# 0xPolygonZero/proof-protocol-decoder

Hardware: NVIDIA B200
Metric: mpt_nodes_keccak_hashed_per_sec (higher is better)
Workload: dtype u64

## Files before the change

proof_protocol_decoder_b200/csrc/gpu_dump.cu:

```cuda
#include "host_pipeline.h"

namespace ppd {

struct LitPool {
  std::vector<uint8_t> b;
  void u8(uint8_t v) { b.push_back(v); }
  void u32(uint32_t v) {
    uint8_t t[4];
    memcpy(t, &v, 4);
    b.insert(b.end(), t, t + 4);
  }
  void raw(const uint8_t* p, size_t n) {
    if (n) b.insert(b.end(), p, p + n);
  }
  void span(Span s) {
    u32(s.n);
    raw(s.p, s.n);
  }
  void u256(uint64_t v) {
    uint8_t be[32];
    memset(be, 0, 32);
    for (int i = 0; i < 8; i++) be[31 - i] = (uint8_t)(v >> (8 * i));
    raw(be, 32);
  }
// ... 88 lines not shown
      t += p.touched.size();
    }
  }
  memcpy(h + o_tb, touched_begin.data(), 4 * (n_ir + 1));
  memcpy(h + o_sa, seg_a.data(), 4 * n_seg);
  memcpy(h + o_sb, seg_b.data(), 4 * n_seg);
  memcpy(h + o_sg, seg_begin.data(), 4 * (n_ir + 1));
  L->d_plan.reserve(4 * o_end);
  uint32_t* d = L->d_plan.as<uint32_t>();
  CUDA_OK(cudaMemcpyAsync(d, h, 4 * o_base, cudaMemcpyHostToDevice, L->st));
  IrDumpPlanView P{};
  P.touched = d + o_touched, P.touched_begin = d + o_tb, P.seg_a = d + o_sa, P.seg_b = d + o_sb, P.seg_begin = d + o_sg;
  P.ir_base = reinterpret_cast<const uint64_t*>(d + o_base);
  P.seg_off = d + o_soff, P.ir_size = d + o_isz, P.ir_flag = d + o_ifl, P.ir_nuniq = d + o_inu;
  P.u_node = d + o_un, P.u_size = d + o_us, P.u_off = d + o_uo;
  pt.lap("  d:plan");
  launch_ir_size(L->last_view, P, n_ir, L->st);
  CUDA_OK(cudaGetLastError());
  CUDA_OK(cudaMemcpyAsync(h + o_soff, d + o_soff, 4 * (o_inu - o_soff), cudaMemcpyDeviceToHost, L->st));
  lane_sync(L);
  L->stats.h2d_bytes += 4.0 * o_base, L->stats.d2h_bytes += 4.0 * (o_inu - o_soff), L->stats.kernel_launches += 1;
  pt.lap("  d:size");
  const uint32_t *seg_off = h + o_soff, *ir_size = h + o_isz;
  uint32_t* ir_flag = h + o_ifl;
  std::vector<Out> host_parts(n_ir);
  Stamp st;
  uint64_t* ir_base = reinterpret_cast<uint64_t*>(h + o_base);
  uint64_t total = 8;
  for (uint32_t i = 0; i < n_ir; i++) {
    ir_base[i] = total;
// ... 91 lines not shown
```

proof_protocol_decoder_b200/csrc/gpu_txn.cu:

```cuda
#include "host_pipeline.h"
#include "txn_tables.h"

namespace ppd {

bool gpu_txn_enabled() {
#ifdef PPD_HOSTPROF
  return false;
#else
  return gpu_parse_enabled() && gpu_dump_enabled() && getenv("PPD_HOST_TXN") == nullptr;
#endif
}

struct LoopBatcher {
  static const int MAX_STREAMS = 16, BMAX = (int)LOOP_BATCH_MAX;
  struct Req {
    txn::LoopTask task;
    uint32_t n_txns = 0;
    cudaEvent_t ready = nullptr, start = nullptr, done = nullptr, done_blocking = nullptr;
    bool launched = false;
    uint32_t launches = 0;
    cudaError_t err = cudaSuccess;
  };
  struct LoopStream {
    cudaStream_t st = nullptr;
// ... 371 lines not shown
    P.ir_nuniq = cv.take<uint32_t>(n_ir + 1);
    d_big_off = cv.take<uint64_t>(n_ir + 1), d_big_cap = cv.take<uint32_t>(n_ir + 1);
    P.big_scratch = cv.take<uint32_t>(big_words + 16);
    P.u_node = cv.take<uint32_t>((size_t)n_touched + 16), P.u_size = cv.take<uint32_t>((size_t)n_touched + 16), P.u_off = cv.take<uint32_t>((size_t)n_touched + 16);
  };
  {
    Carve2 sz{nullptr};
    plan_layout(sz);
    L->d_plan.reserve(sz.off + 256);
    Carve2 cv{L->d_plan.as<uint8_t>()};
    plan_layout(cv);
  }
  P.ir_size = d_ir_size, P.ir_flag = d_ir_size + n_ir;
  P.touched = d_touched, P.touched_begin = d_touched_begin, P.seg_a = d_seg_a, P.seg_b = d_seg_b, P.seg_c = d_seg_c, P.seg_begin = d_seg_begin;
  P.seg_end = d_seg_end;
  P.big_off = d_big_off, P.big_cap = d_big_cap;
  P.flat = d_flat, P.lit = d_lit, P.ir_base = d_ir_base;
  auto up = [&](void* dst, const void* src, size_t bytes) {
    if (!bytes) return;
    lane_copy(L, dst, src, bytes);
    L->stats.h2d_bytes += (double)bytes;
  };
  up(d_txns, T.txns.data(), sizeof(txn::TxnDesc) * T.txns.size());
  up(d_seg_a, T.seg_a.data(), 4ull * n_seg), up(d_seg_b, T.seg_b.data(), 4ull * n_seg), up(d_seg_c, T.seg_c.data(), 4ull * n_seg);
  up(d_touched_begin, T.touched_begin.data(), 4ull * (n_ir + 1));
  if (!n_dummies) up(d_seg_begin, T.seg_begin.data(), 4ull * (n_ir + 1)), up(d_seg_end, T.seg_end.data(), 4ull * (n_ir + 1));
  up(d_lit, T.lit.data(), T.lit.size());
  up(d_big_off, big_off.data(), 8ull * n_ir), up(d_big_cap, big_cap.data(), 4ull * n_ir);
  up(v.key_pool + H.B.txn_key_base, T.txn_keys.data(), T.txn_keys.size());
  lane_copy_flush(L);
  CUDA_OK(cudaMemsetAsync(d_touched, 0xff, 4ull * n_touched, st));
// ... 242 lines not shown
```

proof_protocol_decoder_b200/csrc/ppd_dump.cu:

```cuda
#include <cstddef>
#include <cstdint>

#include "../../include/ppd_flat.h"
#include "arena.h"
#include "ppd_kernels.h"

namespace ppd {

namespace {

constexpr uint32_t HASH_ID_BASE = 0x80000000u;
constexpr uint32_t SET_CAP = 8192, MAX_UNIQ = 4096, NOT_FOUND = 0xffffffffu, UNSET = 0xffffffffu;
#ifndef PPD_DUMP_THREADS
#define PPD_DUMP_THREADS 1024
#endif
constexpr int DUMP_THREADS = PPD_DUMP_THREADS;

struct SharedSet {
  uint32_t key[SET_CAP];
  uint32_t slot[SET_CAP];
  uint32_t u_node[MAX_UNIQ], u_size[MAX_UNIQ], u_off[MAX_UNIQ];
  uint32_t u_par[MAX_UNIQ];
};
struct Set {
  uint32_t *key, *slot, *u_node, *u_size, *u_off, *u_par;
  uint32_t shift, mask, max_uniq;
  uint32_t n_uniq, n_done, flag;
};

__device__ __forceinline__ uint32_t hash_slot(const Set& s, uint32_t id) { return (id * 2654435761u) >> s.shift; }

__device__ __forceinline__ uint32_t set_find(const Set& s, uint32_t id) {
  uint32_t h = hash_slot(s, id);
  for (;;) {
    uint32_t k = s.key[h];
    if (k == id) return s.slot[h];
    if (k == NODE_EMPTY) return NOT_FOUND;
    h = (h + 1) & s.mask;
  }
}

__device__ void set_bind(Set& s, SharedSet& sm, const IrDumpPlanView& P, uint32_t ir, uint32_t tb) {
  if (threadIdx.x == 0) {
    const uint64_t big = P.big_off ? P.big_off[ir] : ~0ull;
    if (big == ~0ull) {
      s.key = sm.key, s.slot = sm.slot, s.u_node = sm.u_node, s.u_size = sm.u_size, s.u_off = sm.u_off, s.u_par = sm.u_par;
      s.mask = SET_CAP - 1, s.shift = 19, s.max_uniq = MAX_UNIQ;
    } else {
      const uint32_t cap = P.big_cap[ir];
      s.key = P.big_scratch + big, s.slot = s.key + cap, s.u_par = s.slot + cap;
      s.u_node = P.u_node + tb, s.u_size = P.u_size + tb, s.u_off = P.u_off + tb;
      s.mask = cap - 1, s.shift = 32 - (31 - __clz(cap)), s.max_uniq = cap / 2;
    }
  }
  __syncthreads();
}

__device__ __forceinline__ bool is_hash_id(uint32_t id) { return id >= HASH_ID_BASE && id != NODE_EMPTY; }
__device__ __forceinline__ uint32_t node_kind(const ArenaView& A, uint32_t id) { return A.nodes[id].w0 & 0xff; }

__device__ __forceinline__ uint32_t u256_sig(const uint8_t* be) {
  uint32_t i = 0;
  while (i < 32 && be[i] == 0) i++;
  return 32 - i;
}
__device__ __forceinline__ uint32_t u256_str_len(const uint8_t* be, uint32_t sig) { return sig == 0 ? 1u : (sig == 1 && be[31] < 0x80) ? 1u : 1u + sig; }
__device__ __forceinline__ uint32_t account_rlp_len(const AccountRec& r) {
  return 2 + u256_str_len(r.nonce, u256_sig(r.nonce)) + u256_str_len(r.balance, u256_sig(r.balance)) + 66;
}

__device__ __forceinline__ uint32_t child_size(const ArenaView& A, const Set& s, uint32_t c, uint32_t* flag) {
  if (c == NODE_EMPTY) return 1;
  if (is_hash_id(c)) return 33;
  uint32_t k = set_find(s, c);
  if (k != NOT_FOUND) return s.u_size[k];
  if (A.ref_len[c] != 32 && node_kind(A, c) != NK_ROOT) *flag = 1;
  return 33;
}

// ... 15 lines not shown
      for (uint32_t j = 0; j < k; j++) {
        uint32_t cs = child_size(A, s, A.child_pool[r.a0 + j], flag);
        if (cs == UNSET) return UNSET;
        total += cs;
      }
      return total;
    }
    default:
      *flag = 1;
      return 33;
  }
}

__device__ void build_set(Set& s, const uint32_t* ids, uint32_t n, const ArenaView& A, bool dedupe) {
  for (uint32_t i = threadIdx.x; i <= s.mask; i += blockDim.x) s.key[i] = NODE_EMPTY;
  if (threadIdx.x == 0) s.n_uniq = 0, s.n_done = 0, s.flag = 0;
  __syncthreads();
  for (uint32_t i = threadIdx.x; i < n; i += blockDim.x) {
    uint32_t id = ids[i];
    if (id == NODE_EMPTY || is_hash_id(id)) continue;
    if (dedupe && node_kind(A, id) == NK_ROOT) continue;
    uint32_t h = hash_slot(s, id);
    for (;;) {
      uint32_t prev = atomicCAS(&s.key[h], NODE_EMPTY, id);
      if (prev == NODE_EMPTY) {
        uint32_t k = dedupe ? atomicAdd(&s.n_uniq, 1u) : i;
        if (k < s.max_uniq) {
          s.slot[h] = k;
          s.u_node[k] = id;
        } else {
          s.flag = 1;
          s.slot[h] = 0;
        }
        break;
      }
      if (prev == id) break;
      h = (h + 1) & s.mask;
    }
  }
  __syncthreads();
}

}

__global__ void __launch_bounds__(DUMP_THREADS) ir_size_kernel(ArenaView A, IrDumpPlanView P) {
  extern __shared__ uint8_t smem_raw[];
  __shared__ Set s;
  const uint32_t ir = blockIdx.x;
  const uint32_t tb = P.touched_begin[ir], tn = P.touched_begin[ir + 1] - tb;
  set_bind(s, *reinterpret_cast<SharedSet*>(smem_raw), P, ir, tb);
  build_set(s, P.touched + tb, tn, A, true);
  const uint32_t nu = min(s.n_uniq, s.max_uniq);
  constexpr uint32_t PLACED = 0x80000000u, NO_KIDS = 0x40000000u;
  for (uint32_t k = threadIdx.x; k < nu; k += blockDim.x) s.u_par[k] = UNSET;
  __syncthreads();
  {
    uint32_t local_flag = 0;
    for (uint32_t k = threadIdx.x; k < nu; k += blockDim.x) {
      const NodeRec r = A.nodes[s.u_node[k]];
      const uint32_t kind = r.w0 & 0xff, nlen = (r.w0 >> 16) & 0xff;
      uint32_t fixed = 0, pend = 0;
      auto child = [&](uint32_t c) {
        if (c == NODE_EMPTY) return 1u;
        if (is_hash_id(c)) return 33u;
        const uint32_t kc = set_find(s, c);
        if (kc != NOT_FOUND) {
          if (atomicCAS(&s.u_par[kc], UNSET, k) != UNSET) local_flag = 1;
          pend++;
          return 0u;
        }
        if (A.ref_len[c] != 32 && node_kind(A, c) != NK_ROOT) local_flag = 1;
        return 33u;
      };
      switch (kind) {
        case NK_LEAF:
          fixed = 1 + 1 + nlen + 4 + r.a2;
          break;
        case NK_LEAF_ACCOUNT:
          fixed = 1 + 1 + nlen + 4 + account_rlp_len(A.accounts[r.a1]);
          break;
        case NK_EXT:
          fixed = 1 + 1 + nlen + child(r.a1);
          break;
        case NK_BRANCH: {
          const uint32_t mask = r.a1 & 0xffff, nk = __popc(mask);
          uint32_t cid[16];
#pragma unroll
          for (uint32_t j = 0; j < 16; j++) cid[j] = j < nk ? A.child_pool[r.a0 + j] : NODE_EMPTY;
          fixed = 1 + (16 - nk) + 4;
#pragma unroll
          for (uint32_t j = 0; j < 16; j++)
            if (j < nk) fixed += child(cid[j]);
          break;
        }
        default:
          local_flag = 1;
          fixed = 33;
      }
      s.u_size[k] = fixed;
      s.u_off[k] = pend ? pend : NO_KIDS;
    }
    if (local_flag) s.flag = 1;
  }
  __syncthreads();
  for (uint32_t k = threadIdx.x; k < nu; k += blockDim.x) {
    if (s.u_off[k] != NO_KIDS) continue;
    uint32_t cur = k;
    for (uint32_t guard = 0; guard < 128; guard++) {
      const uint32_t p = s.u_par[cur];
      if (p == UNSET) break;
      atomicAdd(&s.u_size[p], *reinterpret_cast<volatile uint32_t*>(&s.u_size[cur]));
      __threadfence_block();
      if (atomicSub(&s.u_off[p], 1u) != 1u) break;
      __threadfence_block();
      cur = p;
// ... 60 lines not shown
      if (q < se) {
        P.seg_off[q] = off;
        if (trie_slot != NOT_FOUND && atomicCAS(&s.u_off[trie_slot], UNSET, off) != UNSET) s.flag = 1;
      }
      __syncthreads();
      if (threadIdx.x == DUMP_THREADS - 1) scan_carry = off + sz;
      __syncthreads();
    }
    if (threadIdx.x == 0) {
      P.ir_size[ir] = scan_carry;
      s.n_done = 0;
    }
  }
  __syncthreads();
  if (!s.flag) {
    for (uint32_t k = threadIdx.x; k < nu; k += blockDim.x) {
      const NodeRec r = A.nodes[s.u_node[k]];
      const uint32_t kind = r.w0 & 0xff, nlen = (r.w0 >> 16) & 0xff;
      if (kind == NK_EXT) {
        const uint32_t c = is_hash_id(r.a1) ? NOT_FOUND : set_find(s, r.a1);
        if (c != NOT_FOUND) {
          if (s.u_off[c] != UNSET) s.flag = 1;
          s.u_off[c] = 2 + nlen;
        }
      } else if (kind == NK_BRANCH) {
        const uint32_t mask = r.a1 & 0xffff, nk = __popc(mask);
        uint32_t cid[16];
#pragma unroll
        for (uint32_t j = 0; j < 16; j++) cid[j] = j < nk ? A.child_pool[r.a0 + j] : NODE_EMPTY;
        uint32_t off = 1;
        for (uint32_t i = 0, j = 0; i < 16; i++) {
          if (!(mask & (1u << i))) {
            off += 1;
            continue;
          }
          uint32_t c_id = NODE_EMPTY;
#pragma unroll
          for (uint32_t z = 0; z < 16; z++)
            if (z == j) c_id = cid[z];
          j++;
          const uint32_t c = is_hash_id(c_id) ? NOT_FOUND : set_find(s, c_id);
          if (c != NOT_FOUND) {
            if (s.u_off[c] != UNSET) s.flag = 1;
            s.u_off[c] = off;
            off += s.u_size[c];
          } else {
            off += 33;
          }
        }
      }
    }
  }
  __syncthreads();
  for (int round = 0; round < 130; round++) {
    __syncthreads();
    if (s.flag || s.n_done >= nu) break;
    __syncthreads();
    uint32_t progressed = 0;
    for (uint32_t k = threadIdx.x; k < nu; k += blockDim.x) {
      if (*reinterpret_cast<volatile uint32_t*>(&s.u_size[k]) & PLACED) continue;
      const uint32_t p = s.u_par[k];
      uint32_t off = *reinterpret_cast<volatile uint32_t*>(&s.u_off[k]);
      if (p != UNSET) {
// ... 31 lines not shown
  const uint32_t w[8] = {x.x, x.y, x.z, x.w, y.x, y.y, y.z, y.w};
  uint32_t S[10];
  S[0] = (uint32_t)PPD_NODE_HASH | (w[0] << 8);
#pragma unroll
  for (int k = 1; k < 8; k++) S[k] = __funnelshift_r(w[k - 1], w[k], 24);
  S[8] = w[7] >> 24;
  S[9] = 0;
  const uint32_t head = (4u - (uint32_t)(reinterpret_cast<uintptr_t>(q) & 3u)) & 3u;
  for (uint32_t i = 0; i < head; i++) q[i] = (uint8_t)(S[0] >> (8 * i));
  uint32_t* qw = reinterpret_cast<uint32_t*>(q + head);
  const uint32_t sh = 8 * head, nwords = (33u - head) >> 2;
#pragma unroll
  for (int j = 0; j < 8; j++)
    if ((uint32_t)j < nwords) qw[j] = __funnelshift_r(S[j], S[j + 1], sh);
  const uint32_t done = head + 4 * nwords;
  for (uint32_t i = done; i < 33; i++) q[i] = (uint8_t)(S[i >> 2] >> (8 * (i & 3)));
  return q + 33;
}
__device__ __forceinline__ uint8_t* put_hash(uint8_t* q, const uint8_t* h32) {
  const uint4* src = reinterpret_cast<const uint4*>(h32);
  return put_hash_regs(q, __ldg(src), __ldg(src + 1));
}
__device__ __forceinline__ uint8_t* put_u32(uint8_t* q, uint32_t v) {
  q[0] = (uint8_t)v, q[1] = (uint8_t)(v >> 8), q[2] = (uint8_t)(v >> 16), q[3] = (uint8_t)(v >> 24);
  return q + 4;
}
__device__ __forceinline__ uint8_t* put_nibbles(uint8_t* q, const ArenaView& A, const NodeRec& r) {
  const uint32_t start = (r.w0 >> 8) & 0xff, n = (r.w0 >> 16) & 0xff;
  const uint8_t* key = A.key_pool + r.a0;
  *q++ = (uint8_t)n;
  for (uint32_t i = 0; i < n; i++) {
    uint32_t b = key[(start + i) >> 1];
    *q++ = (uint8_t)(((start + i) & 1) ? (b & 15) : (b >> 4));
  }
  return q;
}
__device__ __forceinline__ uint8_t* put_u256_str(uint8_t* q, const uint8_t* be) {
  uint32_t sig = u256_sig(be);
  if (sig == 0) {
    *q++ = 0x80;
    return q;
  }
  if (!(sig == 1 && be[31] < 0x80)) *q++ = (uint8_t)(0x80 + sig);
  for (uint32_t i = 32 - sig; i < 32; i++) *q++ = be[i];
  return q;
}
__device__ __forceinline__ uint8_t* put_child(uint8_t* q, const ArenaView& A, const Set& s, uint32_t c) {
  if (c == NODE_EMPTY) {
    *q++ = PPD_NODE_EMPTY;
    return q;
  }
  if (is_hash_id(c)) return put_hash(q, A.hash_pool + 32ull * (c - HASH_ID_BASE));
  uint32_t k = set_find(s, c);
  if (k != NOT_FOUND) return q + s.u_size[k];
  return put_hash(q, A.ref + 32ull * c);
}

}

__device__ void emit_node(const ArenaView& A, const Set& s, uint32_t u, uint8_t* q) {
  const NodeRec r = A.nodes[u];
  switch (r.w0 & 0xff) {
    case NK_LEAF: {
      *q++ = PPD_NODE_LEAF;
      q = put_nibbles(q, A, r);
      q = put_u32(q, r.a2);
      const uint8_t* v = A.val_pool + r.a1;
      for (uint32_t i = 0; i < r.a2; i++) q[i] = v[i];
      break;
    }
    case NK_LEAF_ACCOUNT: {
      const AccountRec& acc = A.accounts[r.a1];
      *q++ = PPD_NODE_LEAF;
      q = put_nibbles(q, A, r);
      uint32_t len = account_rlp_len(acc);
      q = put_u32(q, len);
      *q++ = 0xf8;
      *q++ = (uint8_t)(len - 2);
      q = put_u256_str(q, acc.nonce);
      q = put_u256_str(q, acc.balance);
      const uint8_t* sr = acc.storage_src == NODE_EMPTY ? acc.storage_root : A.ref + 32ull * acc.storage_src;
      *q++ = 0xa0;
      for (int i = 0; i < 32; i++) *q++ = sr[i];
      *q++ = 0xa0;
      for (int i = 0; i < 32; i++) *q++ = acc.code_hash[i];
      break;
    }
    case NK_EXT:
      *q++ = PPD_NODE_EXTENSION;
      q = put_nibbles(q, A, r);
      put_child(q, A, s, r.a1);
      break;
    case NK_BRANCH: {
      *q++ = PPD_NODE_BRANCH;
      const uint32_t mask = r.a1 & 0xffff, nk = __popc(mask);
      uint32_t cid[16];
#pragma unroll
      for (uint32_t j = 0; j < 16; j++) cid[j] = j < nk ? A.child_pool[r.a0 + j] : NODE_EMPTY;
      uint32_t m = mask;
      int prev_slot = -1;
#pragma unroll
      for (uint32_t g = 0; g < 16; g += 4) {
        if (g >= nk) break;
        const uint4* src[4];
        uint32_t skip[4];
        uint4 x[4], y[4];
#pragma unroll
        for (uint32_t z = 0; z < 4; z++) {
          const uint32_t c = cid[g + z];
          src[z] = nullptr, skip[z] = 0;
          if (g + z >= nk) continue;
          if (c == NODE_EMPTY) {
            skip[z] = NOT_FOUND;
          } else if (is_hash_id(c)) {
            src[z] = reinterpret_cast<const uint4*>(A.hash_pool + 32ull * (c - HASH_ID_BASE));
          } else {
            const uint32_t k = set_find(s, c);
            if (k != NOT_FOUND)
              skip[z] = s.u_size[k];
            else
              src[z] = reinterpret_cast<const uint4*>(A.ref + 32ull * c);
          }
        }
#pragma unroll
        for (uint32_t z = 0; z < 4; z++)
          if (src[z]) x[z] = __ldg(src[z]), y[z] = __ldg(src[z] + 1);
#pragma unroll
        for (uint32_t z = 0; z < 4; z++) {
          if (g + z >= nk) continue;
          const int slot = __ffs((int)m) - 1;
          m &= m - 1;
          for (int e = prev_slot + 1; e < slot; e++) *q++ = PPD_NODE_EMPTY;
          prev_slot = slot;
          if (src[z])
            q = put_hash_regs(q, x[z], y[z]);
          else if (skip[z] == NOT_FOUND)
            *q++ = PPD_NODE_EMPTY;
          else
            q += skip[z];
        }
      }
      for (int e = prev_slot + 1; e < 16; e++) *q++ = PPD_NODE_EMPTY;
      put_u32(q, 0);
      break;
    }
    default:
      break;
  }
}

__global__ void __launch_bounds__(DUMP_THREADS) ir_emit_kernel(ArenaView A, IrDumpPlanView P, uint8_t* __restrict__ out) {
  extern __shared__ uint8_t smem_raw[];
  __shared__ Set s;
  const uint32_t ir = blockIdx.x;
  if (P.ir_flag[ir]) return;
  const uint32_t tb = P.touched_begin[ir], nu = P.ir_nuniq[ir];
  set_bind(s, *reinterpret_cast<SharedSet*>(smem_raw), P, ir, tb);
  if (s.u_node != P.u_node + tb) {
    build_set(s, P.u_node + tb, nu, A, false);
    for (uint32_t k = threadIdx.x; k < nu; k += blockDim.x) s.u_size[k] = P.u_size[tb + k], s.u_off[k] = P.u_off[tb + k];
  }
  __syncthreads();
  uint8_t* base = out + P.ir_base[ir];
  for (uint32_t k = threadIdx.x; k < nu; k += blockDim.x) emit_node(A, s, s.u_node[k], base + s.u_off[k]);
  const uint32_t sb = P.seg_begin[ir], se = P.seg_end ? P.seg_end[ir] : P.seg_begin[ir + 1];
  for (uint32_t qi = sb + threadIdx.x; qi < se; qi += blockDim.x) {
    const uint32_t b = P.seg_b[qi];
    if (b == IR_SEG_LITERAL) continue;
    uint8_t* q = base + P.seg_off[qi];
    if (b == IR_SEG_REF || b == IR_SEG_KEY32) {
      const uint8_t* r = b == IR_SEG_REF ? A.ref + 32ull * P.seg_a[qi] : A.key_pool + P.seg_a[qi];
      for (int i = 0; i < 32; i++) q[i] = r[i];
      continue;
    }
    if (b == IR_SEG_ROOT_ONLY) {
      const uint32_t a = P.seg_a[qi];
      if (a == NODE_EMPTY)
        *q = PPD_NODE_EMPTY;
      else if (is_hash_id(a))
        put_hash(q, A.hash_pool + 32ull * (a - HASH_ID_BASE));
      else if (node_kind(A, a) == NK_ROOT)
        put_hash(q, A.ref + 32ull * a);
      else
        emit_node(A, s, a, q);
      continue;
    }
    if (b == IR_SEG_FLAT || b == IR_SEG_LIT_DEV) {
      const uint32_t len = P.seg_a[qi];
      if (len > 96) continue;
      const uint8_t* src = (b == IR_SEG_FLAT ? P.flat : P.lit) + P.seg_c[qi];
      for (uint32_t i = 0; i < len; i++) q[i] = src[i];
      continue;
    }
    if (b == NODE_EMPTY)
      *q = PPD_NODE_EMPTY;
    else if (is_hash_id(b))
      put_hash(q, A.hash_pool + 32ull * (b - HASH_ID_BASE));
    else if (set_find(s, b) == NOT_FOUND)
      put_hash(q, A.ref + 32ull * b);
  }
  if (P.seg_c) {
    for (uint32_t qi = sb; qi < se; qi++) {
      const uint32_t b = P.seg_b[qi];
      if (b != IR_SEG_FLAT && b != IR_SEG_LIT_DEV) continue;
      const uint32_t len = P.seg_a[qi];
      if (len <= 96) continue;
      const uint8_t* src = (b == IR_SEG_FLAT ? P.flat : P.lit) + P.seg_c[qi];
      uint8_t* q = base + P.seg_off[qi];
      for (uint32_t i = threadIdx.x; i < len; i += blockDim.x) q[i] = src[i];
    }
  }
}

size_t ir_dump_smem_bytes() { return sizeof(SharedSet); }

void launch_ir_size(const ArenaView& A, const IrDumpPlanView& P, uint32_t n_ir, cudaStream_t st) {
  if (!n_ir) return;
  static bool attr = false;
  if (!attr) {
    cudaFuncSetAttribute(ir_size_kernel, cudaFuncAttributeMaxDynamicSharedMemorySize, (int)sizeof(SharedSet));
    cudaFuncSetAttribute(ir_emit_kernel, cudaFuncAttributeMaxDynamicSharedMemorySize, (int)sizeof(SharedSet));
    attr = true;
  }
  ir_size_kernel<<<n_ir, DUMP_THREADS, sizeof(SharedSet), st>>>(A, P);
}
void launch_ir_emit(const ArenaView& A, const IrDumpPlanView& P, uint32_t n_ir, uint8_t* out, cudaStream_t st) {
  if (!n_ir) return;
  ir_emit_kernel<<<n_ir, DUMP_THREADS, offsetof(SharedSet, u_par), st>>>(A, P, out);
}

}
```

proof_protocol_decoder_b200/csrc/ppd_kernels.h:

```cpp
#pragma once
#include <cuda_runtime.h>

#include <cstdint>

#include "arena.h"
#include "txn_core.h"

namespace ppd {

void launch_keccak256_batch(const uint8_t* data, const uint64_t* offsets, uint32_t n, uint8_t* out, cudaStream_t st);
void launch_keccak256_ranges(const uint8_t* data, const uint64_t* begin_end, uint32_t n, uint8_t* out, cudaStream_t st);
void launch_hash_level(const ArenaView& A, const uint32_t* order, uint32_t begin, uint32_t end, cudaStream_t st);
static const uint32_t ORDER_MAX_BINS = 4096;
void launch_order_by_level_class(const NodeRec* nodes, const uint16_t* level, uint32_t n, uint32_t n_bins, uint16_t* keys, uint32_t* bins,
                                 uint32_t* order, cudaStream_t st, uint32_t first = 0, const uint32_t* n_dev = nullptr);

struct CopyBatch {
  static const uint32_t MAX = 16;
  void* dst[MAX];
  const void* src[MAX];
  unsigned long long bytes[MAX];
  uint32_t n = 0;
};
void launch_copy_segments(const CopyBatch& B, cudaStream_t st);
// ... 45 lines not shown

struct IrDumpPlanView {
  const uint32_t* touched;
  const uint32_t* touched_begin;
  const uint32_t* seg_a;
  const uint32_t* seg_b;
  const uint32_t* seg_begin;
  const uint32_t* seg_end;
  const uint32_t* seg_c;
  const uint8_t* flat;
  const uint8_t* lit;
  const uint64_t* ir_base;
  const uint64_t* big_off;
  const uint32_t* big_cap;
  uint32_t* big_scratch;
  uint32_t* seg_off;
  uint32_t* ir_size;
  uint32_t* ir_flag;
  uint32_t* ir_nuniq;
  uint32_t* u_node;
  uint32_t* u_size;
  uint32_t* u_off;
};
void launch_ir_size(const ArenaView& A, const IrDumpPlanView& P, uint32_t n_ir, cudaStream_t st);
static const uint32_t MARK_SLOTS = 16;
static const uint32_t IR_SET_MAX_UNIQ = 4096;
void launch_ir_emit(const ArenaView& A, const IrDumpPlanView& P, uint32_t n_ir, uint8_t* out, cudaStream_t st);

static const uint32_t PARSE_TILE = 4096;
static const uint32_t PARSE_ERR = 0xffffff00u;
enum {
  PARSE_R_END = 0,
  PARSE_R_NINS = 1,
  PARSE_R_FLAG = 2,
  PARSE_R_HEIGHT = 3,
  PARSE_R_ROOT = 4,
  PARSE_R_ROOT_ID = 5,
  PARSE_R_NKEYED = 6,
  PARSE_R_TOTALS = 8,
  PARSE_R_WORDS = 16
};
// ... 80 lines not shown
```

Measured before the change: 1.460 billion.

## Process dump nodes with 16-lane groups and size shared-memory sets to the workload

The IR size and emit kernels now work on each trie node with a 16-thread half-warp instead of one thread per node. Branch children are handled one per lane with warp reduce and scan, and account RLP bytes are written cooperatively. The shared-memory hash set is sized from the largest per-IR touched count, with 512 threads and two blocks per SM. IRs that overflow the small set are flagged and rerun in a second wide launch. This targets per-thread serial work and low occupancy from the fixed large shared allocation, at the cost of extra launches, redo passes and more complex control flow.

```diff
diff --git a/profiles/dump_times.py b/profiles/dump_times.py
--- /dev/null
+++ b/profiles/dump_times.py
@@ -0,0 +1,72 @@
+#!/usr/bin/env python3
+import argparse
+import json
+import os
+import statistics
+import subprocess
+import sys
+
+HERE = os.path.dirname(os.path.dirname(os.path.abspath(__file__)))
+
+
+def main():
+    ap = argparse.ArgumentParser()
+    ap.add_argument("--root", default=HERE)
+    ap.add_argument("--reps", type=int, default=50)
+    ap.add_argument("--lanes", type=int, default=30)
+    ap.add_argument("--out", default=None)
+    args = ap.parse_args()
+    sys.dont_write_bytecode = True
+    sys.path.insert(0, os.path.abspath(args.root))
+    sys.path.insert(1, HERE)
+    os.environ.setdefault("PPD_HOST_THREADS", str(max(args.lanes, 1)))
+    import torch
+
+    import bench
+    from proof_protocol_decoder_b200.lib import Context
+
+    flats = bench.c2_blocks([2 + j for j in range(args.lanes)], 1.0, os.cpu_count() or 1)
+    ctx = Context(0)
+    flush = torch.empty(256 << 20, dtype=torch.uint8, device="cuda")
+    gpu = subprocess.run(["nvidia-smi", "--query-gpu=name,power.limit", "--format=csv,noheader"], capture_output=True, text=True).stdout.strip()
+    result = {"root": os.path.abspath(args.root), "gpu": gpu, "reps": args.reps}
+
+    def events(reps):
+        for _ in range(5):
+            ctx.replay_last(ctx.REPLAY_DUMP)
+        ms = []
+        for _ in range(reps):
+            flush.zero_()
+            torch.cuda.synchronize()
+            ms.append(ctx.replay_last(ctx.REPLAY_DUMP))
+        return {"mean_ms": statistics.mean(ms), "median_ms": statistics.median(ms), "min_ms": min(ms), "max_ms": max(ms)}
+
+    def kernels(reps):
+        from torch.profiler import ProfilerActivity, profile
+
+        with profile(activities=[ProfilerActivity.CUDA]) as prof:
+            for _ in range(reps):
+                ctx.replay_last(ctx.REPLAY_DUMP)
+            torch.cuda.synchronize()
+        out = {}
+        for e in prof.events():
+            for k in ("ir_size_kernel", "ir_emit_kernel"):
+                if k in e.name and e.device_type.name == "CUDA":
+                    out.setdefault(k, []).append(e.device_time_total if hasattr(e, "device_time_total") else e.cuda_time_total)
+        return {k: {"launches": len(v), "mean_us": statistics.mean(v), "per_replay_us": sum(v) / reps} for k, v in out.items()}
+
+    ctx.block_decode(flats[0])
+    assert ctx.stats()["txn_loops_on_gpu"] == 1, "the block's txn loop did not run on the device: no dump to replay"
+    result["one_block"] = {"lanes": ctx.replay_lanes(), "replay": events(args.reps), "kernels": kernels(args.reps)}
+    got = []
+    for _ in range(2):
+        ctx.blocks_decode_stream(flats, lambda i, o: (got.append(o.nbytes), o.close()))
+    result["concurrent"] = {"lanes": ctx.replay_lanes(), "replay": events(args.reps), "kernels": kernels(args.reps)}
+    print(json.dumps(result, indent=1))
+    if args.out:
+        with open(args.out, "w") as f:
+            json.dump(result, f, indent=1)
+
+
+if __name__ == "__main__":
+    main()
diff --git a/proof_protocol_decoder_b200/csrc/gpu_dump.cu b/proof_protocol_decoder_b200/csrc/gpu_dump.cu
--- a/proof_protocol_decoder_b200/csrc/gpu_dump.cu
+++ b/proof_protocol_decoder_b200/csrc/gpu_dump.cu
@@ -126,6 +126,7 @@
   P.ir_base = reinterpret_cast<const uint64_t*>(d + o_base);
   P.seg_off = d + o_soff, P.ir_size = d + o_isz, P.ir_flag = d + o_ifl, P.ir_nuniq = d + o_inu;
   P.u_node = d + o_un, P.u_size = d + o_us, P.u_off = d + o_uo;
+  P.set_uniq = ir_set_uniq(touched_begin.data(), n_ir, nullptr);
   pt.lap("  d:plan");
   launch_ir_size(L->last_view, P, n_ir, L->st);
   CUDA_OK(cudaGetLastError());
diff --git a/proof_protocol_decoder_b200/csrc/gpu_txn.cu b/proof_protocol_decoder_b200/csrc/gpu_txn.cu
--- a/proof_protocol_decoder_b200/csrc/gpu_txn.cu
+++ b/proof_protocol_decoder_b200/csrc/gpu_txn.cu
@@ -409,7 +409,7 @@
   P.ir_size = d_ir_size, P.ir_flag = d_ir_size + n_ir;
   P.touched = d_touched, P.touched_begin = d_touched_begin, P.seg_a = d_seg_a, P.seg_b = d_seg_b, P.seg_c = d_seg_c, P.seg_begin = d_seg_begin;
   P.seg_end = d_seg_end;
-  P.big_off = d_big_off, P.big_cap = d_big_cap;
+  P.big_off = d_big_off, P.big_cap = d_big_cap, P.set_uniq = ir_set_uniq(T.touched_begin.data(), n_ir, big_off.data());
   P.flat = d_flat, P.lit = d_lit, P.ir_base = d_ir_base;
   auto up = [&](void* dst, const void* src, size_t bytes) {
     if (!bytes) return;
diff --git a/proof_protocol_decoder_b200/csrc/ppd_dump.cu b/proof_protocol_decoder_b200/csrc/ppd_dump.cu
--- a/proof_protocol_decoder_b200/csrc/ppd_dump.cu
+++ b/proof_protocol_decoder_b200/csrc/ppd_dump.cu
@@ -1,3 +1,4 @@
+#include <algorithm>
 #include <cstddef>
 #include <cstdint>
 
@@ -10,22 +11,33 @@
 namespace {
 
 constexpr uint32_t HASH_ID_BASE = 0x80000000u;
-constexpr uint32_t SET_CAP = 8192, MAX_UNIQ = 4096, NOT_FOUND = 0xffffffffu, UNSET = 0xffffffffu;
-#ifndef PPD_DUMP_THREADS
-#define PPD_DUMP_THREADS 1024
-#endif
-constexpr int DUMP_THREADS = PPD_DUMP_THREADS;
-
-struct SharedSet {
-  uint32_t key[SET_CAP];
-  uint32_t slot[SET_CAP];
-  uint32_t u_node[MAX_UNIQ], u_size[MAX_UNIQ], u_off[MAX_UNIQ];
-  uint32_t u_par[MAX_UNIQ];
+constexpr uint32_t MAX_UNIQ = IR_SET_MAX_UNIQ, NOT_FOUND = 0xffffffffu, UNSET = 0xffffffffu;
+constexpr int DUMP_THREADS = 512, DUMP_MIN_BLOCKS = 2;
+constexpr uint32_t GROUPS = DUMP_THREADS / 16;
+
+constexpr uint32_t SMALL_UNIQ = 1280, IR_REDO = 2;
+struct SetDims {
+  uint32_t cap, uniq;
 };
+__host__ __device__ inline SetDims set_dims(uint32_t set_uniq) {
+  const uint32_t uniq = set_uniq < 1 ? 1 : set_uniq > MAX_UNIQ ? MAX_UNIQ : set_uniq;
+  uint32_t cap = 32;
+  while (cap < 2 * uniq) cap <<= 1;
+  return {cap, uniq};
+}
+inline size_t size_smem_bytes(uint32_t set_uniq) {
+  const SetDims d = set_dims(set_uniq);
+  return 4ull * (2 * d.cap + 4 * d.uniq);
+}
+inline size_t emit_smem_bytes(uint32_t set_uniq) {
+  const SetDims d = set_dims(set_uniq);
+  return 4ull * (2 * d.cap + d.uniq);
+}
+
 struct Set {
   uint32_t *key, *slot, *u_node, *u_size, *u_off, *u_par;
   uint32_t shift, mask, max_uniq;
-  uint32_t n_uniq, n_done, flag;
+  uint32_t n_uniq, n_done, flag, redo;
 };
 
 __device__ __forceinline__ uint32_t hash_slot(const Set& s, uint32_t id) { return (id * 2654435761u) >> s.shift; }
@@ -40,12 +52,14 @@
   }
 }
 
-__device__ void set_bind(Set& s, SharedSet& sm, const IrDumpPlanView& P, uint32_t ir, uint32_t tb) {
+__device__ bool set_bind(Set& s, uint32_t* sm, const IrDumpPlanView& P, uint32_t ir, uint32_t tb, uint32_t uniq) {
+  const uint64_t big = P.big_off ? P.big_off[ir] : ~0ull;
   if (threadIdx.x == 0) {
-    const uint64_t big = P.big_off ? P.big_off[ir] : ~0ull;
     if (big == ~0ull) {
-      s.key = sm.key, s.slot = sm.slot, s.u_node = sm.u_node, s.u_size = sm.u_size, s.u_off = sm.u_off, s.u_par = sm.u_par;
-      s.mask = SET_CAP - 1, s.shift = 19, s.max_uniq = MAX_UNIQ;
+      const SetDims d = set_dims(uniq);
+      s.key = sm, s.slot = sm + d.cap, s.u_size = s.slot + d.cap, s.u_node = s.u_size + d.uniq, s.u_off = s.u_node + d.uniq;
+      s.u_par = s.u_off + d.uniq;
+      s.mask = d.cap - 1, s.shift = 32 - (31 - __clz(d.cap)), s.max_uniq = d.uniq;
     } else {
       const uint32_t cap = P.big_cap[ir];
       s.key = P.big_scratch + big, s.slot = s.key + cap, s.u_par = s.slot + cap;
@@ -54,6 +68,7 @@
     }
   }
   __syncthreads();
+  return big != ~0ull;
 }
 
 __device__ __forceinline__ bool is_hash_id(uint32_t id) { return id >= HASH_ID_BASE && id != NODE_EMPTY; }
@@ -63,6 +78,13 @@
   uint32_t i = 0;
   while (i < 32 && be[i] == 0) i++;
   return 32 - i;
+}
+__device__ __forceinline__ uint32_t u256_sig16(const uint8_t* be, uint32_t lane, uint32_t hmask) {
+  const uint32_t b0 = be[2 * lane], b1 = be[2 * lane + 1];
+  const uint32_t nz = (__ballot_sync(hmask, (b0 | b1) != 0) >> (threadIdx.x & 16)) & 0xffffu;
+  const uint32_t f = nz ? __ffs((int)nz) - 1 : 0;
+  const uint32_t first = __shfl_sync(hmask, b0, f, 16);
+  return nz ? 32 - (2 * f + (first == 0)) : 0;
 }
 __device__ __forceinline__ uint32_t u256_str_len(const uint8_t* be, uint32_t sig) { return sig == 0 ? 1u : (sig == 1 && be[31] < 0x80) ? 1u : 1u + sig; }
 __device__ __forceinline__ uint32_t account_rlp_len(const AccountRec& r) {
@@ -108,22 +130,27 @@
 
 __device__ void build_set(Set& s, const uint32_t* ids, uint32_t n, const ArenaView& A, bool dedupe) {
   for (uint32_t i = threadIdx.x; i <= s.mask; i += blockDim.x) s.key[i] = NODE_EMPTY;
-  if (threadIdx.x == 0) s.n_uniq = 0, s.n_done = 0, s.flag = 0;
+  if (threadIdx.x == 0) s.n_uniq = 0, s.n_done = 0, s.flag = 0, s.redo = 0;
   __syncthreads();
   for (uint32_t i = threadIdx.x; i < n; i += blockDim.x) {
+    if (*reinterpret_cast<volatile uint32_t*>(&s.redo)) break;
     uint32_t id = ids[i];
     if (id == NODE_EMPTY || is_hash_id(id)) continue;
     if (dedupe && node_kind(A, id) == NK_ROOT) continue;
     uint32_t h = hash_slot(s, id);
-    for (;;) {
+    for (uint32_t probe = 0;; probe++) {
+      if (probe > s.mask) {
+        s.flag = 1, s.redo = 1;
+        break;
+      }
       uint32_t prev = atomicCAS(&s.key[h], NODE_EMPTY, id);
       if (prev == NODE_EMPTY) {
         uint32_t k = dedupe ? atomicAdd(&s.n_uniq, 1u) : i;
         if (k < s.max_uniq) {
           s.slot[h] = k;
-          s.u_node[k] = id;
+          if (dedupe) s.u_node[k] = id;
         } else {
-          s.flag = 1;
+          s.flag = 1, s.redo = 1;
           s.slot[h] = 0;
         }
         break;
@@ -135,64 +162,86 @@
   __syncthreads();
 }
 
-}
-
-__global__ void __launch_bounds__(DUMP_THREADS) ir_size_kernel(ArenaView A, IrDumpPlanView P) {
-  extern __shared__ uint8_t smem_raw[];
+__device__ __forceinline__ uint32_t scan16(uint32_t v, uint32_t lane, uint32_t hmask) {
+#pragma unroll
+  for (int o = 1; o < 16; o <<= 1) {
+    const uint32_t t = __shfl_up_sync(hmask, v, o, 16);
+    if (lane >= (uint32_t)o) v += t;
+  }
+  return v;
+}
+
+__device__ __forceinline__ uint32_t branch_slot_child(const ArenaView& A, const NodeRec& r, uint32_t lane) {
+  const uint32_t mask = r.a1 & 0xffff;
+  if (!((mask >> lane) & 1)) return NODE_EMPTY;
+  return A.child_pool[r.a0 + __popc(mask & ((1u << lane) - 1))];
+}
+
+}
+
+__global__ void __launch_bounds__(DUMP_THREADS, DUMP_MIN_BLOCKS) ir_size_kernel(ArenaView A, IrDumpPlanView P, bool wide) {
+  extern __shared__ uint32_t smem_words[];
   __shared__ Set s;
   const uint32_t ir = blockIdx.x;
+  if (wide && P.ir_flag[ir] != IR_REDO) return;
   const uint32_t tb = P.touched_begin[ir], tn = P.touched_begin[ir + 1] - tb;
-  set_bind(s, *reinterpret_cast<SharedSet*>(smem_raw), P, ir, tb);
+  const uint32_t lane = threadIdx.x & 15, grp = threadIdx.x >> 4, hmask = 0xffffu << (threadIdx.x & 16);
+  const bool big = set_bind(s, smem_words, P, ir, tb, wide ? P.set_uniq : min(P.set_uniq, SMALL_UNIQ));
   build_set(s, P.touched + tb, tn, A, true);
+  if (!wide && !big && s.redo && P.set_uniq > SMALL_UNIQ) {
+    if (threadIdx.x == 0) P.ir_flag[ir] = IR_REDO;
+    return;
+  }
   const uint32_t nu = min(s.n_uniq, s.max_uniq);
   constexpr uint32_t PLACED = 0x80000000u, NO_KIDS = 0x40000000u;
   for (uint32_t k = threadIdx.x; k < nu; k += blockDim.x) s.u_par[k] = UNSET;
   __syncthreads();
   {
     uint32_t local_flag = 0;
-    for (uint32_t k = threadIdx.x; k < nu; k += blockDim.x) {
+    auto child = [&](uint32_t c, uint32_t k, uint32_t& pend) {
+      if (c == NODE_EMPTY) return 1u;
+      if (is_hash_id(c)) return 33u;
+      const uint32_t kc = set_find(s, c);
+      if (kc != NOT_FOUND) {
+        if (atomicCAS(&s.u_par[kc], UNSET, k) != UNSET) local_flag = 1;
+        pend++;
+        return 0u;
+      }
+      if (A.ref_len[c] != 32 && node_kind(A, c) != NK_ROOT) local_flag = 1;
+      return 33u;
+    };
+    for (uint32_t k = grp; k < nu; k += GROUPS) {
       const NodeRec r = A.nodes[s.u_node[k]];
       const uint32_t kind = r.w0 & 0xff, nlen = (r.w0 >> 16) & 0xff;
       uint32_t fixed = 0, pend = 0;
-      auto child = [&](uint32_t c) {
-        if (c == NODE_EMPTY) return 1u;
-        if (is_hash_id(c)) return 33u;
-        const uint32_t kc = set_find(s, c);
-        if (kc != NOT_FOUND) {
-          if (atomicCAS(&s.u_par[kc], UNSET, k) != UNSET) local_flag = 1;
-          pend++;
-          return 0u;
-        }
-        if (A.ref_len[c] != 32 && node_kind(A, c) != NK_ROOT) local_flag = 1;
-        return 33u;
-      };
       switch (kind) {
         case NK_LEAF:
           fixed = 1 + 1 + nlen + 4 + r.a2;
           break;
-        case NK_LEAF_ACCOUNT:
-          fixed = 1 + 1 + nlen + 4 + account_rlp_len(A.accounts[r.a1]);
+        case NK_LEAF_ACCOUNT: {
+          const AccountRec& acc = A.accounts[r.a1];
+          fixed = 1 + 1 + nlen + 4 + 2 + u256_str_len(acc.nonce, u256_sig16(acc.nonce, lane, hmask)) +
+                  u256_str_len(acc.balance, u256_sig16(acc.balance, lane, hmask)) + 66;
           break;
+        }
         case NK_EXT:
-          fixed = 1 + 1 + nlen + child(r.a1);
+          if (lane == 0) fixed = 1 + 1 + nlen + child(r.a1, k, pend);
           break;
         case NK_BRANCH: {
           const uint32_t mask = r.a1 & 0xffff, nk = __popc(mask);
-          uint32_t cid[16];
-#pragma unroll
-          for (uint32_t j = 0; j < 16; j++) cid[j] = j < nk ? A.child_pool[r.a0 + j] : NODE_EMPTY;
-          fixed = 1 + (16 - nk) + 4;
-#pragma unroll
-          for (uint32_t j = 0; j < 16; j++)
-            if (j < nk) fixed += child(cid[j]);
+          const uint32_t part = lane < nk ? child(A.child_pool[r.a0 + lane], k, pend) : 0u;
+          const uint32_t both = __reduce_add_sync(hmask, part | (pend << 16));
+          fixed = 1 + (16 - nk) + 4 + (both & 0xffff), pend = both >> 16;
           break;
         }
         default:
           local_flag = 1;
           fixed = 33;
       }
-      s.u_size[k] = fixed;
-      s.u_off[k] = pend ? pend : NO_KIDS;
+      if (lane == 0) {
+        s.u_size[k] = fixed;
+        s.u_off[k] = pend ? pend : NO_KIDS;
+      }
     }
     if (local_flag) s.flag = 1;
   }
@@ -283,39 +332,23 @@
   }
   __syncthreads();
   if (!s.flag) {
-    for (uint32_t k = threadIdx.x; k < nu; k += blockDim.x) {
+    for (uint32_t k = grp; k < nu; k += GROUPS) {
       const NodeRec r = A.nodes[s.u_node[k]];
       const uint32_t kind = r.w0 & 0xff, nlen = (r.w0 >> 16) & 0xff;
       if (kind == NK_EXT) {
-        const uint32_t c = is_hash_id(r.a1) ? NOT_FOUND : set_find(s, r.a1);
+        const uint32_t c = (lane != 0 || r.a1 == NODE_EMPTY || is_hash_id(r.a1)) ? NOT_FOUND : set_find(s, r.a1);
         if (c != NOT_FOUND) {
           if (s.u_off[c] != UNSET) s.flag = 1;
           s.u_off[c] = 2 + nlen;
         }
       } else if (kind == NK_BRANCH) {
-        const uint32_t mask = r.a1 & 0xffff, nk = __popc(mask);
-        uint32_t cid[16];
-#pragma unroll
-        for (uint32_t j = 0; j < 16; j++) cid[j] = j < nk ? A.child_pool[r.a0 + j] : NODE_EMPTY;
-        uint32_t off = 1;
-        for (uint32_t i = 0, j = 0; i < 16; i++) {
-          if (!(mask & (1u << i))) {
-            off += 1;
-            continue;
-          }
-          uint32_t c_id = NODE_EMPTY;
-#pragma unroll
-          for (uint32_t z = 0; z < 16; z++)
-            if (z == j) c_id = cid[z];
-          j++;
-          const uint32_t c = is_hash_id(c_id) ? NOT_FOUND : set_find(s, c_id);
-          if (c != NOT_FOUND) {
-            if (s.u_off[c] != UNSET) s.flag = 1;
-            s.u_off[c] = off;
-            off += s.u_size[c];
-          } else {
-            off += 33;
-          }
+        const uint32_t c_id = branch_slot_child(A, r, lane);
+        const uint32_t c = (c_id == NODE_EMPTY || is_hash_id(c_id)) ? NOT_FOUND : set_find(s, c_id);
+        const uint32_t sz = c_id == NODE_EMPTY ? 1u : c != NOT_FOUND ? s.u_size[c] : 33u;
+        const uint32_t off = 1 + scan16(sz, lane, hmask) - sz;
+        if (c != NOT_FOUND) {
+          if (s.u_off[c] != UNSET) s.flag = 1;
+          s.u_off[c] = off;
         }
       }
     }
@@ -377,16 +410,14 @@
   for (int j = 0; j < 8; j++)
     if ((uint32_t)j < nwords) qw[j] = __funnelshift_r(S[j], S[j + 1], sh);
   const uint32_t done = head + 4 * nwords;
-  for (uint32_t i = done; i < 33; i++) q[i] = (uint8_t)(S[i >> 2] >> (8 * (i & 3)));
+  if (done <= 30) q[30] = (uint8_t)(S[7] >> 16);
+  if (done <= 31) q[31] = (uint8_t)(S[7] >> 24);
+  if (done <= 32) q[32] = (uint8_t)S[8];
   return q + 33;
 }
 __device__ __forceinline__ uint8_t* put_hash(uint8_t* q, const uint8_t* h32) {
   const uint4* src = reinterpret_cast<const uint4*>(h32);
   return put_hash_regs(q, __ldg(src), __ldg(src + 1));
-}
-__device__ __forceinline__ uint8_t* put_u32(uint8_t* q, uint32_t v) {
-  q[0] = (uint8_t)v, q[1] = (uint8_t)(v >> 8), q[2] = (uint8_t)(v >> 16), q[3] = (uint8_t)(v >> 24);
-  return q + 4;
 }
 __device__ __forceinline__ uint8_t* put_nibbles(uint8_t* q, const ArenaView& A, const NodeRec& r) {
   const uint32_t start = (r.w0 >> 8) & 0xff, n = (r.w0 >> 16) & 0xff;
@@ -398,16 +429,6 @@
   }
   return q;
 }
-__device__ __forceinline__ uint8_t* put_u256_str(uint8_t* q, const uint8_t* be) {
-  uint32_t sig = u256_sig(be);
-  if (sig == 0) {
-    *q++ = 0x80;
-    return q;
-  }
-  if (!(sig == 1 && be[31] < 0x80)) *q++ = (uint8_t)(0x80 + sig);
-  for (uint32_t i = 32 - sig; i < 32; i++) *q++ = be[i];
-  return q;
-}
 __device__ __forceinline__ uint8_t* put_child(uint8_t* q, const ArenaView& A, const Set& s, uint32_t c) {
   if (c == NODE_EMPTY) {
     *q++ = PPD_NODE_EMPTY;
@@ -419,114 +440,136 @@
   return put_hash(q, A.ref + 32ull * c);
 }
 
-}
-
-__device__ void emit_node(const ArenaView& A, const Set& s, uint32_t u, uint8_t* q) {
+__device__ __forceinline__ uint8_t leaf_head_byte(const ArenaView& A, const NodeRec& r, uint32_t vlen, uint32_t t) {
+  const uint32_t start = (r.w0 >> 8) & 0xff, n = (r.w0 >> 16) & 0xff;
+  if (t == 0) return PPD_NODE_LEAF;
+  if (t == 1) return (uint8_t)n;
+  if (t < 2 + n) {
+    const uint32_t i = start + t - 2, b = A.key_pool[r.a0 + (i >> 1)];
+    return (uint8_t)((i & 1) ? (b & 15) : (b >> 4));
+  }
+  return (uint8_t)(vlen >> (8 * (t - 2 - n)));
+}
+__device__ __forceinline__ uint8_t u256_str_byte(const uint8_t* be, uint32_t sig, uint32_t p) {
+  if (sig == 0) return 0x80;
+  if (sig == 1 && be[31] < 0x80) return be[31];
+  return p == 0 ? (uint8_t)(0x80 + sig) : be[32 - sig + p - 1];
+}
+
+__device__ __forceinline__ void copy16(uint8_t* dst, const uint8_t* src, uint32_t n, uint32_t lane) {
+  const uint32_t head = min(n, (4u - (uint32_t)(reinterpret_cast<uintptr_t>(dst) & 3u)) & 3u);
+  if (lane < head) dst[lane] = src[lane];
+  const uint32_t nw = (n - head) >> 2;
+  const uint8_t* s0 = src + head;
+  const uint32_t sh = 8 * (uint32_t)(reinterpret_cast<uintptr_t>(s0) & 3u);
+  const uint32_t* sw = reinterpret_cast<const uint32_t*>(reinterpret_cast<uintptr_t>(s0) & ~(uintptr_t)3);
+  uint32_t* dw = reinterpret_cast<uint32_t*>(dst + head);
+  for (uint32_t w = lane; w < nw; w += 16) dw[w] = sh ? __funnelshift_r(sw[w], sw[w + 1], sh) : sw[w];
+  const uint32_t done = head + 4 * nw;
+  if (done + lane < n) dst[done + lane] = src[done + lane];
+}
+
+__device__ void emit_node16(const ArenaView& A, const Set& s, uint32_t u, uint8_t* q, uint32_t lane, uint32_t hmask) {
   const NodeRec r = A.nodes[u];
   switch (r.w0 & 0xff) {
+    case NK_BRANCH: {
+      const uint32_t c = branch_slot_child(A, r, lane);
+      const uint4* src = nullptr;
+      uint32_t sz = 1;
+      if (c != NODE_EMPTY) {
+        sz = 33;
+        if (is_hash_id(c)) {
+          src = reinterpret_cast<const uint4*>(A.hash_pool + 32ull * (c - HASH_ID_BASE));
+        } else {
+          const uint32_t k = set_find(s, c);
+          if (k != NOT_FOUND)
+            sz = s.u_size[k];
+          else
+            src = reinterpret_cast<const uint4*>(A.ref + 32ull * c);
+        }
+      }
+      uint4 x = make_uint4(0, 0, 0, 0), y = x;
+      if (src) x = __ldg(src), y = __ldg(src + 1);
+      const uint32_t incl = scan16(sz, lane, hmask), total = __shfl_sync(hmask, incl, 15, 16);
+      uint8_t* p = q + 1 + incl - sz;
+      if (src)
+        put_hash_regs(p, x, y);
+      else if (c == NODE_EMPTY)
+        *p = PPD_NODE_EMPTY;
+      if (lane == 0) *q = PPD_NODE_BRANCH;
+      if (lane < 4) q[1 + total + lane] = 0;
+      break;
+    }
     case NK_LEAF: {
-      *q++ = PPD_NODE_LEAF;
-      q = put_nibbles(q, A, r);
-      q = put_u32(q, r.a2);
-      const uint8_t* v = A.val_pool + r.a1;
-      for (uint32_t i = 0; i < r.a2; i++) q[i] = v[i];
+      const uint32_t head = 6 + ((r.w0 >> 16) & 0xff);
+      for (uint32_t t = lane; t < head; t += 16) q[t] = leaf_head_byte(A, r, r.a2, t);
+      copy16(q + head, A.val_pool + r.a1, r.a2, lane);
       break;
     }
     case NK_LEAF_ACCOUNT: {
       const AccountRec& acc = A.accounts[r.a1];
-      *q++ = PPD_NODE_LEAF;
-      q = put_nibbles(q, A, r);
-      uint32_t len = account_rlp_len(acc);
-      q = put_u32(q, len);
-      *q++ = 0xf8;
-      *q++ = (uint8_t)(len - 2);
-      q = put_u256_str(q, acc.nonce);
-      q = put_u256_str(q, acc.balance);
+      const uint32_t head = 6 + ((r.w0 >> 16) & 0xff);
+      const uint32_t nsig = u256_sig16(acc.nonce, lane, hmask), bsig = u256_sig16(acc.balance, lane, hmask);
+      const uint32_t nl = u256_str_len(acc.nonce, nsig), bl = u256_str_len(acc.balance, bsig), len = 2 + nl + bl + 66;
       const uint8_t* sr = acc.storage_src == NODE_EMPTY ? acc.storage_root : A.ref + 32ull * acc.storage_src;
-      *q++ = 0xa0;
-      for (int i = 0; i < 32; i++) *q++ = sr[i];
-      *q++ = 0xa0;
-      for (int i = 0; i < 32; i++) *q++ = acc.code_hash[i];
+      for (uint32_t t = lane; t < head + len; t += 16) {
+        uint8_t v;
+        if (t < head) {
+          v = leaf_head_byte(A, r, len, t);
+        } else {
+          uint32_t p = t - head;
+          if (p < 2) {
+            v = p == 0 ? 0xf8 : (uint8_t)(len - 2);
+          } else if ((p -= 2) < nl) {
+            v = u256_str_byte(acc.nonce, nsig, p);
+          } else if ((p -= nl) < bl) {
+            v = u256_str_byte(acc.balance, bsig, p);
+          } else {
+            p -= bl;
+            v = (p == 0 || p == 33) ? 0xa0 : p < 33 ? sr[p - 1] : acc.code_hash[p - 34];
+          }
+        }
+        q[t] = v;
+      }
       break;
     }
     case NK_EXT:
-      *q++ = PPD_NODE_EXTENSION;
-      q = put_nibbles(q, A, r);
-      put_child(q, A, s, r.a1);
+      if (lane == 0) {
+        *q++ = PPD_NODE_EXTENSION;
+        q = put_nibbles(q, A, r);
+        put_child(q, A, s, r.a1);
+      }
       break;
-    case NK_BRANCH: {
-      *q++ = PPD_NODE_BRANCH;
-      const uint32_t mask = r.a1 & 0xffff, nk = __popc(mask);
-      uint32_t cid[16];
-#pragma unroll
-      for (uint32_t j = 0; j < 16; j++) cid[j] = j < nk ? A.child_pool[r.a0 + j] : NODE_EMPTY;
-      uint32_t m = mask;
-      int prev_slot = -1;
-#pragma unroll
-      for (uint32_t g = 0; g < 16; g += 4) {
-        if (g >= nk) break;
-        const uint4* src[4];
-        uint32_t skip[4];
-        uint4 x[4], y[4];
-#pragma unroll
-        for (uint32_t z = 0; z < 4; z++) {
-          const uint32_t c = cid[g + z];
-          src[z] = nullptr, skip[z] = 0;
-          if (g + z >= nk) continue;
-          if (c == NODE_EMPTY) {
-            skip[z] = NOT_FOUND;
-          } else if (is_hash_id(c)) {
-            src[z] = reinterpret_cast<const uint4*>(A.hash_pool + 32ull * (c - HASH_ID_BASE));
-          } else {
-            const uint32_t k = set_find(s, c);
-            if (k != NOT_FOUND)
-              skip[z] = s.u_size[k];
-            else
-              src[z] = reinterpret_cast<const uint4*>(A.ref + 32ull * c);
-          }
-        }
-#pragma unroll
-        for (uint32_t z = 0; z < 4; z++)
-          if (src[z]) x[z] = __ldg(src[z]), y[z] = __ldg(src[z] + 1);
-#pragma unroll
-        for (uint32_t z = 0; z < 4; z++) {
-          if (g + z >= nk) continue;
-          const int slot = __ffs((int)m) - 1;
-          m &= m - 1;
-          for (int e = prev_slot + 1; e < slot; e++) *q++ = PPD_NODE_EMPTY;
-          prev_slot = slot;
-          if (src[z])
-            q = put_hash_regs(q, x[z], y[z]);
-          else if (skip[z] == NOT_FOUND)
-            *q++ = PPD_NODE_EMPTY;
-          else
-            q += skip[z];
-        }
-      }
-      for (int e = prev_slot + 1; e < 16; e++) *q++ = PPD_NODE_EMPTY;
-      put_u32(q, 0);
-      break;
-    }
     default:
       break;
   }
 }
 
-__global__ void __launch_bounds__(DUMP_THREADS) ir_emit_kernel(ArenaView A, IrDumpPlanView P, uint8_t* __restrict__ out) {
-  extern __shared__ uint8_t smem_raw[];
+}
+
+__global__ void __launch_bounds__(DUMP_THREADS, DUMP_MIN_BLOCKS) ir_emit_kernel(ArenaView A, IrDumpPlanView P, uint8_t* __restrict__ out, bool wide) {
+  extern __shared__ uint32_t smem_words[];
   __shared__ Set s;
   const uint32_t ir = blockIdx.x;
   if (P.ir_flag[ir]) return;
   const uint32_t tb = P.touched_begin[ir], nu = P.ir_nuniq[ir];
-  set_bind(s, *reinterpret_cast<SharedSet*>(smem_raw), P, ir, tb);
-  if (s.u_node != P.u_node + tb) {
+  const uint32_t lane = threadIdx.x & 15, grp = threadIdx.x >> 4, hmask = 0xffffu << (threadIdx.x & 16);
+  const bool big = P.big_off && P.big_off[ir] != ~0ull;
+  if (wide != (!big && nu > SMALL_UNIQ)) return;
+  if (!set_bind(s, smem_words, P, ir, tb, wide ? P.set_uniq : min(P.set_uniq, SMALL_UNIQ))) {
     build_set(s, P.u_node + tb, nu, A, false);
-    for (uint32_t k = threadIdx.x; k < nu; k += blockDim.x) s.u_size[k] = P.u_size[tb + k], s.u_off[k] = P.u_off[tb + k];
-  }
-  __syncthreads();
+    for (uint32_t k = threadIdx.x; k < nu; k += blockDim.x) s.u_size[k] = P.u_size[tb + k];
+    __syncthreads();
+  }
+  const uint32_t *u_node = P.u_node + tb, *u_off = P.u_off + tb;
   uint8_t* base = out + P.ir_base[ir];
-  for (uint32_t k = threadIdx.x; k < nu; k += blockDim.x) emit_node(A, s, s.u_node[k], base + s.u_off[k]);
+  for (uint32_t k = grp; k < nu; k += GROUPS) emit_node16(A, s, u_node[k], base + u_off[k], lane, hmask);
   const uint32_t sb = P.seg_begin[ir], se = P.seg_end ? P.seg_end[ir] : P.seg_begin[ir + 1];
+  for (uint32_t qi = sb + grp; qi < se; qi += GROUPS) {
+    if (P.seg_b[qi] != IR_SEG_ROOT_ONLY) continue;
+    const uint32_t a = P.seg_a[qi];
+    if (a != NODE_EMPTY && !is_hash_id(a) && node_kind(A, a) != NK_ROOT) emit_node16(A, s, a, base + P.seg_off[qi], lane, hmask);
+  }
   for (uint32_t qi = sb + threadIdx.x; qi < se; qi += blockDim.x) {
     const uint32_t b = P.seg_b[qi];
     if (b == IR_SEG_LITERAL) continue;
@@ -544,8 +587,6 @@
         put_hash(q, A.hash_pool + 32ull * (a - HASH_ID_BASE));
       else if (node_kind(A, a) == NK_ROOT)
         put_hash(q, A.ref + 32ull * a);
-      else
-        emit_node(A, s, a, q);
       continue;
     }
     if (b == IR_SEG_FLAT || b == IR_SEG_LIT_DEV) {
@@ -575,21 +616,28 @@
   }
 }
 
-size_t ir_dump_smem_bytes() { return sizeof(SharedSet); }
+uint32_t ir_set_uniq(const uint32_t* touched_begin, uint32_t n_ir, const uint64_t* big_off) {
+  uint32_t m = 0;
+  for (uint32_t i = 0; i < n_ir; i++)
+    if (!big_off || big_off[i] == ~0ull) m = std::max(m, touched_begin[i + 1] - touched_begin[i]);
+  return std::min(m, MAX_UNIQ);
+}
 
 void launch_ir_size(const ArenaView& A, const IrDumpPlanView& P, uint32_t n_ir, cudaStream_t st) {
   if (!n_ir) return;
   static bool attr = false;
   if (!attr) {
-    cudaFuncSetAttribute(ir_size_kernel, cudaFuncAttributeMaxDynamicSharedMemorySize, (int)sizeof(SharedSet));
-    cudaFuncSetAttribute(ir_emit_kernel, cudaFuncAttributeMaxDynamicSharedMemorySize, (int)sizeof(SharedSet));
+    cudaFuncSetAttribute(ir_size_kernel, cudaFuncAttributeMaxDynamicSharedMemorySize, (int)size_smem_bytes(MAX_UNIQ));
+    cudaFuncSetAttribute(ir_emit_kernel, cudaFuncAttributeMaxDynamicSharedMemorySize, (int)emit_smem_bytes(MAX_UNIQ));
     attr = true;
   }
-  ir_size_kernel<<<n_ir, DUMP_THREADS, sizeof(SharedSet), st>>>(A, P);
+  ir_size_kernel<<<n_ir, DUMP_THREADS, size_smem_bytes(std::min(P.set_uniq, SMALL_UNIQ)), st>>>(A, P, false);
+  if (P.set_uniq > SMALL_UNIQ) ir_size_kernel<<<n_ir, DUMP_THREADS, size_smem_bytes(P.set_uniq), st>>>(A, P, true);
 }
 void launch_ir_emit(const ArenaView& A, const IrDumpPlanView& P, uint32_t n_ir, uint8_t* out, cudaStream_t st) {
   if (!n_ir) return;
-  ir_emit_kernel<<<n_ir, DUMP_THREADS, offsetof(SharedSet, u_par), st>>>(A, P, out);
-}
-
-}
+  ir_emit_kernel<<<n_ir, DUMP_THREADS, emit_smem_bytes(std::min(P.set_uniq, SMALL_UNIQ)), st>>>(A, P, out, false);
+  if (P.set_uniq > SMALL_UNIQ) ir_emit_kernel<<<n_ir, DUMP_THREADS, emit_smem_bytes(P.set_uniq), st>>>(A, P, out, true);
+}
+
+}
diff --git a/proof_protocol_decoder_b200/csrc/ppd_kernels.h b/proof_protocol_decoder_b200/csrc/ppd_kernels.h
--- a/proof_protocol_decoder_b200/csrc/ppd_kernels.h
+++ b/proof_protocol_decoder_b200/csrc/ppd_kernels.h
@@ -83,6 +83,7 @@
   const uint64_t* big_off;
   const uint32_t* big_cap;
   uint32_t* big_scratch;
+  uint32_t set_uniq;
   uint32_t* seg_off;
   uint32_t* ir_size;
   uint32_t* ir_flag;
@@ -94,6 +95,7 @@
 void launch_ir_size(const ArenaView& A, const IrDumpPlanView& P, uint32_t n_ir, cudaStream_t st);
 static const uint32_t MARK_SLOTS = 16;
 static const uint32_t IR_SET_MAX_UNIQ = 4096;
+uint32_t ir_set_uniq(const uint32_t* touched_begin, uint32_t n_ir, const uint64_t* big_off);
 void launch_ir_emit(const ArenaView& A, const IrDumpPlanView& P, uint32_t n_ir, uint8_t* out, cudaStream_t st);
 
 static const uint32_t PARSE_TILE = 4096;
```

Measured after the change: 1.460 billion (median of 6 runs). No clear change (+0.0%).
